# LiWentomng/OrientedRepPoints

Hardware: NVIDIA H100
Metric: 1024x1024 tiles/sec (higher is better)
Workload: dtype f16x3

## Files before the change

orientedreppoints_b200/_lib.py:

```python
import ctypes
import os

_HERE = os.path.dirname(os.path.abspath(__file__))
LIB_PATH = os.path.join(_HERE, "lib", "liborp_b200.so")

ORP_NMS_EXACT64, ORP_NMS_COMPAT32 = 0, 1
ORP_UNION_NAN_KEEPS, ORP_UNION_GUARD, ORP_UNION_NAN_SUPPRESSES, ORP_UNION_NAN_SUPPRESSES_ALL = 0, 1, 2, 3
ORP_ORDER_INDEX_ASC, ORP_ORDER_SCORE_DESC = 0, 1
ORP_MERGE_BAD_COUNT, ORP_MERGE_BAD_TILE, ORP_MERGE_ROWS_OVERFLOW = 1, 2, 4

_vp = ctypes.c_void_p
_i = ctypes.c_int
_f = ctypes.c_float
_d = ctypes.c_double


class NmsStats(ctypes.Structure):
    _fields_ = [("pairs_total", ctypes.c_int64), ("pairs_aabb", ctypes.c_int64),
                ("pairs_clipped", ctypes.c_int64), ("pairs_fp64", ctypes.c_int64),
                ("edges", ctypes.c_int64), ("suppressing", ctypes.c_int64), ("overflow", ctypes.c_int32),
                ("rounds", ctypes.c_int32), ("n", ctypes.c_int32)]

    def as_dict(self):
        return {k: int(getattr(self, k)) for k, _ in self._fields_}
# ... 101 lines not shown
    "orp_stem_s2d_u8_padded_bf16": (_i, [_vp, _i, _i, _i, _vp, _vp, _i, _vp, _vp, _vp]),
    "orp_stem_s2d_u8_padded_f16x3": (_i, [_vp, _i, _i, _i, _vp, _vp, _i, _vp, _vp, _vp]),
    "orp_patch_embed_rows_u8_padded_bf16": (_i, [_vp, _i, _i, _i, _vp, _vp, _i, _vp, _vp, _vp]),
    "orp_patch_embed_rows_u8_padded_f16x3": (_i, [_vp, _i, _i, _i, _vp, _vp, _i, _vp, _vp, _vp]),
    "orp_stem_s2d_u8_bf16": (_i, [_vp, _i, _i, _i, _vp, _vp, _i, _vp, _vp]),
    "orp_stem_conv_s2d_bf16": (_i, [_vp, _i, _i, _i, _vp, _vp, _i, _vp, _vp]),
    "orp_maxpool3x3s2_bf16": (_i, [_vp, _i, _i, _i, _i, _vp, _vp]),
    "orp_gn_stats_bf16": (_i, [_vp, _i, _i, _i, _i, _vp, _vp]),
    "orp_gn_apply_bf16_multi": (_i, [_i, _vp, _i, _i, _vp, _vp, _f, _i, _vp]),
}

DCNV2_SIGNATURES = {
    "orp_dcnv2_offset_mask": (_i, [_vp, ctypes.c_longlong, _vp, _vp, _vp]),
}

_LIB = None


class OrpError(RuntimeError):
    pass


def lib():
    global _LIB
    if _LIB is None:
        if not os.path.exists(LIB_PATH):
            raise OrpError(
                "liborp_b200.so not found at %s - build it with `python -m orientedreppoints_b200.build` "
                "(there is no CPU or PyTorch fallback for this path)" % LIB_PATH)
        l = ctypes.CDLL(LIB_PATH)
        for name, (res, args) in list(SIGNATURES.items()) + list(DCNV2_SIGNATURES.items()):
            fn = getattr(l, name)
            fn.restype = res
            fn.argtypes = args
        _LIB = l
    return _LIB


def check(rc, what=""):
    if rc != 0:
        msg = lib().orp_last_error()
        raise OrpError("%s failed (%d): %s" % (what, rc, msg.decode() if msg else ""))


def launch_count():
    return int(lib().orp_launch_count())
# ... 23 lines not shown
    v = ctypes.c_float(0)
    check(lib().orp_rnms_last_sweep_ms(ctypes.byref(v)), "orp_rnms_last_sweep_ms")
    return float(v.value)


def tc_timing_collect():
    ms, n, fl = ctypes.c_float(0), ctypes.c_int(0), ctypes.c_double(0)
    check(lib().orp_tc_timing_collect(ctypes.byref(ms), ctypes.byref(n), ctypes.byref(fl)), "orp_tc_timing_collect")
    return float(ms.value), int(n.value), float(fl.value)


def tc_last_plan():
    p = TcPlan()
    check(lib().orp_tc_last_plan(ctypes.byref(p)), "orp_tc_last_plan")
    return p.as_dict()


def tc_plan_for(problems, cout, cout_p, kh, kw, cin, stride, pad, *, bias=False, relu=0, out_f32=False, deform=False,
                split=False, residual=0, gn=False, stem=0, ksplit=1, sms=132):
    ph = 256
    arr = (TcProblem * len(problems))()
    for q, (n, h, w) in zip(arr, problems):
        q.x, q.N, q.H, q.W, q.out = ph, n, h, w, ph
        q.residual_bf16 = ph if residual == 1 else None
        q.residual_f32 = ph if residual == 2 else None
        q.offset = ph if deform else None
        q.gn_stats = ph if gn else None
    p = TcPlan()
    check(lib().orp_tc_plan_conv(len(problems), arr, ph, cout, cout_p, kh, kw, cin, stride, pad, ph if bias else None, 0,
                                 int(relu), int(out_f32), int(deform), int(split), stem, ksplit, sms, ctypes.byref(p)),
# ... 12 lines not shown
```

orientedreppoints_b200/build.py:

```python
import os
import subprocess
import sys
from concurrent.futures import ThreadPoolExecutor

HERE = os.path.dirname(os.path.abspath(__file__))
CSRC = os.path.join(HERE, "csrc")
OUT = os.path.join(HERE, "lib")
LIB = os.path.join(OUT, "liborp_b200.so")
NVCC = os.environ.get("NVCC", "/usr/local/cuda/bin/nvcc")
ARCH = ["-gencode", "arch=compute_90a,code=sm_90a"]
FLAGS = ["-O3", "-std=c++17", "-lineinfo", "-Xcompiler", "-fPIC", "--expt-relaxed-constexpr",
         "-Xptxas", "-v", "--threads", "2"]


def _sources():
    return sorted(os.path.join(CSRC, f) for f in os.listdir(CSRC) if f.endswith(".cu"))


def _headers():
    hs = [os.path.join(CSRC, f) for f in os.listdir(CSRC) if f.endswith((".cuh", ".h"))]
    hs.append(os.path.join(HERE, "..", "include", "orp_b200.h"))
    hs.append(os.path.join(HERE, "..", "include", "orp_b200_dcnv2.h"))
    return hs


def build(force=False, verbose=False):
    os.makedirs(OUT, exist_ok=True)
    objdir = os.path.join(OUT, "obj")
    os.makedirs(objdir, exist_ok=True)
    hdr_m = max(os.path.getmtime(h) for h in _headers())
    jobs = []
    objs = []
    for src in _sources():
        obj = os.path.join(objdir, os.path.basename(src)[:-3] + ".o")
        objs.append(obj)
        if force or not os.path.exists(obj) or os.path.getmtime(obj) < max(os.path.getmtime(src), hdr_m):
            jobs.append((src, obj))
# ... 30 lines not shown
```

orientedreppoints_b200/csrc/dense_tc.cu:

```cuda
#include <cuda.h>
#include <cuda_bf16.h>
#include <cuda_fp16.h>

#include <cstdlib>
#include <mutex>
#include <type_traits>

#include "common.cuh"
#include "wgmma.cuh"

namespace orp {
namespace {

constexpr int kMaxProb = 5;
constexpr int kStagesMax = 6;
constexpr int kBM = 128;
constexpr int kBK = 64;
constexpr int kABytes = kBM * kBK * 2;

struct FastDiv {
    uint32_t mul, shr, d;
    __host__ void set(uint32_t div)
    {
        d = div;
// ... 12 lines not shown
    int BW, BH, BI;
    int lbw, lbh;
    int tiles_w, tiles_h, tiles_i, tile_start;
    void *out;
    const __nv_bfloat16 *res;
    const float *res32;
    const __nv_bfloat16 *x;
    const float *offset;
    const float *mask;
    double *gn_stats;
};

struct alignas(64) TcParams {
    CUtensorMap tmA[kMaxProb];
    CUtensorMap tmB;
    CUtensorMap tmOut[kMaxProb];
    CUtensorMap tmRes[kMaxProb];
    CUtensorMap tmI;
    Problem prob[kMaxProb];
    int tma_epi, epi_bufs;
    int epi_merge;
    int ncat;
    int ksplit;
    FastDiv fd_ks;
    long long ks_stride;
    int b_resident;
    int res_mma;
    int gn_fused;
    int dcat;
    int split;
    float oscale;
    unsigned int *ovf;
    int nprob, num_m_tiles, n_tiles_n, num_tiles;
    FastDiv fd_ntn;
    int KH, KW, Cin, cin_blocks, stride, pad, Cout, relu;
    int s2d_stem;
    const float *bias;
};

__device__ __forceinline__ uint32_t smem_u32(const void *p) { return (uint32_t)__cvta_generic_to_shared(p); }

__device__ __forceinline__ void mbar_init(uint64_t *bar, uint32_t count)
{
    asm volatile("mbarrier.init.shared::cta.b64 [%0], %1;" ::"r"(smem_u32(bar)), "r"(count));
}
__device__ __forceinline__ void mbar_expect_tx(uint64_t *bar, uint32_t bytes)
{
    asm volatile("mbarrier.arrive.expect_tx.shared::cta.b64 _, [%0], %1;" ::"r"(smem_u32(bar)), "r"(bytes) : "memory");
// ... 31 lines not shown
        "cp.async.bulk.tensor.4d.shared::cluster.global.mbarrier::complete_tx::bytes [%0], [%1, {%3, %4, %5, %6}], [%2];"
        ::"r"(smem_u32(smem)), "l"(tm), "r"(smem_u32(bar)), "r"(c0), "r"(c1), "r"(c2), "r"(c3) : "memory");
}
__device__ __forceinline__ void tma_load_5d(void *smem, const CUtensorMap *tm, uint64_t *bar, int c0, int c1, int c2, int c3, int c4)
{
    asm volatile(
        "cp.async.bulk.tensor.5d.shared::cluster.global.mbarrier::complete_tx::bytes [%0], [%1, {%3, %4, %5, %6, %7}], [%2];"
        ::"r"(smem_u32(smem)), "l"(tm), "r"(smem_u32(bar)), "r"(c0), "r"(c1), "r"(c2), "r"(c3), "r"(c4) : "memory");
}
__device__ __forceinline__ void tma_load_2d(void *smem, const CUtensorMap *tm, uint64_t *bar, int c0, int c1)
{
    asm volatile(
        "cp.async.bulk.tensor.2d.shared::cluster.global.mbarrier::complete_tx::bytes [%0], [%1, {%3, %4}], [%2];"
        ::"r"(smem_u32(smem)), "l"(tm), "r"(smem_u32(bar)), "r"(c0), "r"(c1) : "memory");
}
__device__ __forceinline__ uint64_t make_desc_sw128(uint32_t smem_addr)
{
    uint64_t d = 0;
    d |= (uint64_t)((smem_addr >> 4) & 0x3FFF);
    d |= (uint64_t)1 << 16;
    d |= (uint64_t)(1024 >> 4) << 32;
    d |= (uint64_t)1 << 62;
    return d;
}
__device__ __forceinline__ uint4 lds128(uint32_t addr)
{
    uint4 v;
    asm volatile("ld.shared.v4.b32 {%0, %1, %2, %3}, [%4];" : "=r"(v.x), "=r"(v.y), "=r"(v.z), "=r"(v.w) : "r"(addr) : "memory");
    return v;
}
// ... 89 lines not shown
    uint32_t mt_u, nt_u;
    if (P.ksplit > 1) tile = (int)P.fd_ks.div((uint32_t)tile);
    P.fd_ntn.divmod((uint32_t)tile, mt_u, nt_u);
    nt = (int)nt_u;
    const int mt = (int)mt_u;
    pi = 0;
#pragma unroll
    for (int k = 1; k < kMaxProb; ++k)
        if (k < P.nprob && mt >= P.prob[k].tile_start) pi = k;
    const Problem &pr = P.prob[pi];
    const int local = mt - pr.tile_start;
    uint32_t rest, wb_u, ib_u, hb_u;
    pr.fd_tw.divmod((uint32_t)local, rest, wb_u);
    pr.fd_th.divmod(rest, ib_u, hb_u);
    wb = (int)wb_u; hb = (int)hb_u; ib = (int)ib_u;
}

struct IdentBlock { unsigned short v[64 * 64]; };
constexpr IdentBlock make_ident()
{
    IdentBlock b{};
    for (int i = 0; i < 64; ++i) b.v[i * 64 + i] = 0x3F80;
    return b;
}
__device__ IdentBlock g_ident = make_ident();
struct IdentBlocks16 { unsigned short v[16][64 * 64]; };
constexpr IdentBlocks16 make_ident16()
{
    IdentBlocks16 b{};
    for (int s = 0; s < 16; ++s)
// ... 51 lines not shown
template <int NG, bool BF16, int R, int G = 0>
__device__ __forceinline__ void wgmma_cols64(float (&acc)[R], uint64_t da, uint64_t db, uint32_t accumulate)
{
    wgmma_n<64, BF16>(acc_view<32 * G, 32>(acc), da, db + (uint64_t)(G * 512), accumulate);
    if constexpr (G + 1 < NG) wgmma_cols64<NG, BF16, R, G + 1>(acc, da, db, accumulate);
}

template <int BN, bool BF16>
__device__ __forceinline__ void wgmma_dcat(float (&acc)[BN / 2], uint64_t da, uint64_t db, uint32_t accumulate)
{
    if constexpr (BN == 256) {
        wgmma_n<128, BF16>(acc_view<0, 64>(acc), da, db, accumulate);
        wgmma_n<128, BF16>(acc_view<64, 64>(acc), da, db + (uint64_t)1024, accumulate);
    } else {
        wgmma_n<BN, BF16>(acc, da, db, accumulate);
    }
}

constexpr int kProducerRegs = 40;
constexpr int kConsumerRegs = 232;
constexpr int kWideConsumerRegs = 160;
constexpr int kWideProducerRegs = 96;

template <int BN, bool OUT_F32, bool DEFORM, bool SPLIT, int WALK>
__global__ void __launch_bounds__(DEFORM ? kConsumers + kDP : kConsumers + 128, 1)
conv_tc_kernel(const __grid_constant__ TcParams P, int stages)
{
    static_assert(WALK != kWalkNcat || (SPLIT && !DEFORM && !OUT_F32 && BN >= 64 && BN <= 128), "ncat: f16x3 TMA-epilogue layers, BN 64..128");
    static_assert(!DEFORM || (WALK == kWalkDcat) == SPLIT, "deformable: dcat exactly in f16x3");
    static_assert(DEFORM || WALK != kWalkDcat, "dcat is the deformable walk");
// ... 19 lines not shown
    const int kblocks_all = P.KH * P.KW * P.cin_blocks * kWTerms;
    uint8_t *ident = smem;
    if (P.res_mma) smem += 8192;
    uint8_t *bres = smem;
    if (P.b_resident) smem += (size_t)kblocks_all * kBBytes;
    constexpr int HC = BN < 64 ? BN : 64;
    constexpr int kPitch = HC * 2 + 16;
    uint8_t *stage_out = smem + (size_t)stages * kStageBytes;
    __shared__ uint64_t bars[2 * kStagesMax];
    __shared__ __align__(16) float s_bias[256];
    __shared__ uint64_t bres_bar;
    uint64_t *full = bars;
    uint64_t *empty = bars + kStagesMax;

    const int warp = threadIdx.x >> 5, lane = threadIdx.x & 31;

    if (warp == kConsumers / 32 && elect_one()) {
        if (!DEFORM) {
#pragma unroll 1
            for (int p = 0; p < P.nprob; ++p)
                asm volatile("prefetch.tensormap [%0];" ::"l"(&P.tmA[p]) : "memory");
        }
        asm volatile("prefetch.tensormap [%0];" ::"l"(&P.tmB) : "memory");
    }
    if (warp == 0) {
        if (elect_one()) {
            for (int s = 0; s < stages; ++s) {
                mbar_init(&full[s], DEFORM ? 1 + kDP / 32 : 1);
                mbar_init(&empty[s], kConsumers / 128);
            }
            mbar_init(&bres_bar, 1);
            asm volatile("fence.mbarrier_init.release.cluster;" ::: "memory");
        }
        __syncwarp();
    }
    __syncthreads();
    const int taps_per = (P.KH * P.KW) / (P.ksplit > 1 ? P.ksplit : 1);
    const int kblocks = taps_per * P.cin_blocks * (kKMode ? 3 : 1);
    asm volatile("griddepcontrol.launch_dependents;" ::: "memory");
    asm volatile("griddepcontrol.wait;" ::: "memory");

    if (warp < kConsumers / 32) {
        if constexpr (!DEFORM) setmaxnreg_inc<kConsumerRegs>();
        if constexpr (kFragEpi) setmaxnreg_inc<kWideConsumerRegs>();
        const int cw = warp >> 2;
        const uint32_t a_off = (uint32_t)cw * 8192u;
        const bool leader = (threadIdx.x & 127) == 0;
        float acc[kAccN / 2];
        Ring r(stages);
        const int q = warp & 3, wg = warp >> 2;
        const int et = threadIdx.x, nthr = kEpiThreads;
        const int bar_a = 1, bar_b = 3;
        const int ch0 = wg, chs = kWG;
        const int frow = cw * 64 + (warp & 3) * 16 + (lane >> 2), fcol = 2 * (lane & 3);
        const uint32_t s_acc_u = smem_u32(s_acc);
        auto bar_sync = [](int id, int n) { asm volatile("bar.sync %0, %1;" ::"r"(id), "r"(n) : "memory"); };
        int ob = 0;
        int bias_nt = -1;
        if ((P.b_resident || P.res_mma) && (int)blockIdx.x < P.num_tiles) mbar_wait(&bres_bar, 0);
        for (int tile = blockIdx.x; tile < P.num_tiles; tile += gridDim.x) {
            int res_groups = 0;
            if constexpr (WALK == kWalkKRes) {
                const int nt = tile - (int)P.fd_ntn.div((uint32_t)tile) * P.n_tiles_n;
                for (int g = 0; g < BN / 64 && nt * BN + g * 64 < P.Cout; ++g) ++res_groups;
            }
            const int tap_lo = ksplit_of(P, tile) * taps_per;
            KIter it(tap_lo + taps_per, P.cin_blocks, kKMode, tap_lo);
            int held = -1;
            auto release = [&](int next) {
                if (held >= 0 && leader) mbar_arrive(&empty[held]);
                held = next;
            };
            for (int kb = 0; kb < kblocks; ++kb, it.next()) {
                if constexpr (kFragEpi) {
                    wgmma_wait<0>();
                    release(-1);
                }
                mbar_wait(&full[r.stage], r.phase);
                const uint32_t sa = smem_u32(smem + (size_t)r.stage * kStageBytes);
                const uint64_t da = make_desc_sw128(sa + a_off);
                const int slab = (it.tap * P.cin_blocks + it.cb) * kWTerms + (it.term == 2 ? 1 : 0);
                wgmma_fence();
                if constexpr (WALK == kWalkNcat) {
                    const uint32_t sb = P.b_resident ? smem_u32(bres + (size_t)slab * kBBytes) : sa + 2 * kABytes;
                    const uint64_t dl = make_desc_sw128(sa + kABytes + a_off);
// ... 106 lines not shown
                            if (P.relu) { f0 = fmaxf(f0, 0.f); f1 = fmaxf(f1, 0.f); }
                            if (oterm == 0) amax[hr][i >> 2] = fmaxf(fmaxf(amax[hr][i >> 2], fabsf(f0)), fabsf(f1));
                            const __half2 h2 = __floats2half2_rn(f0, f1);
                            uint32_t v = *reinterpret_cast<const uint32_t *>(&h2);
                            if (oterm) {
                                const float2 hf = __half22float2(h2);
                                const __half2 l2 = __floats2half2_rn(f0 - hf.x, f1 - hf.y);
                                v = *reinterpret_cast<const uint32_t *>(&l2);
                            }
                            const uint32_t at = obase + (uint32_t)row * 128u + ((uint32_t)(i ^ (row & 7)) << 4) + (uint32_t)fcol * 2u;
                            asm volatile("st.shared.b32 [%0], %1;" ::"r"(at), "r"(v) : "memory");
                        }
                    }
                    asm volatile("fence.proxy.async.shared::cta;" ::: "memory");
                    bar_sync(bar_b, nthr);
                    if (io) {
                        asm volatile(
                            "cp.async.bulk.tensor.5d.global.shared::cta.bulk_group [%0, {%2, %3, %4, %5, %6}], [%1];"
                            ::"l"(&P.tmOut[pi]), "r"(obase), "r"(nt * BN + half * 64), "r"(oterm),
                              "r"(wb * pr.BW), "r"(hb * pr.BH), "r"(ib * pr.BI) : "memory");
                        asm volatile("cp.async.bulk.commit_group;" ::: "memory");
                    }
                    if (++ob == P.epi_bufs) ob = 0;
                }
#pragma unroll
                for (int hr = 0; hr < 2; ++hr)
#pragma unroll
                    for (int hc = 0; hc < 2; ++hc) {
                        float m = amax[hr][hc];
                        m = fmaxf(m, __shfl_xor_sync(0xffffffffu, m, 1));
                        m = fmaxf(m, __shfl_xor_sync(0xffffffffu, m, 2));
// ... 128 lines not shown
                                }
                                if (lane == c16) { gn_s = gs; gn_q = gq; }
                            }
                        }
                    }
                    if (P.gn_fused && oterm == 0 && lane < 8 && (chs == 1 || (lane >> 2) == wg)) {
                        const int n_img = ib * pr.BI + ((q * 32) >> (pr.lbw + pr.lbh));
                        if (n_img < pr.N) {
                            double *st = pr.gn_stats + ((size_t)n_img * 32 + (size_t)(nt * BN + half * 64) / 8 + lane) * 2;
                            atomicAdd(st, (double)gn_s);
                            atomicAdd(st + 1, (double)gn_q);
                        }
                    }
                    asm volatile("fence.proxy.async.shared::cta;" ::: "memory");
                    bar_sync(bar_b, nthr);
                    if (io) {
                        asm volatile(
                            "cp.async.bulk.tensor.5d.global.shared::cta.bulk_group [%0, {%2, %3, %4, %5, %6}], [%1];"
                            ::"l"(&P.tmOut[pi]), "r"(obuf_u + (uint32_t)ob * slot), "r"(nt * BN + half * 64), "r"(oterm),
                              "r"(wb * pr.BW), "r"(hb * pr.BH), "r"(ib * pr.BI) : "memory");
                        if (P.epi_merge)
                            asm volatile(
                                "cp.async.bulk.tensor.5d.global.shared::cta.bulk_group [%0, {%2, %3, %4, %5, %6}], [%1];"
                                ::"l"(&P.tmOut[pi]), "r"(obuf_u + (uint32_t)ob * slot + 16384u), "r"(nt * BN + half * 64), "r"(1),
                                  "r"(wb * pr.BW), "r"(hb * pr.BH), "r"(ib * pr.BI) : "memory");
                        asm volatile("cp.async.bulk.commit_group;" ::: "memory");
                    }
                    if (++ob == P.epi_bufs) ob = 0;
                }
                if (P.split && valid && amax > 65504.f) atomicAdd(P.ovf, 1u);
            } else {
// ... 77 lines not shown
                            } else {
                                const __nv_bfloat16 *e8 = reinterpret_cast<const __nv_bfloat16 *>(&u);
                                for (int j = 0; j < 8; ++j) if (cbase + k16 * 8 + j < P.Cout) op[j] = e8[j];
                            }
                        }
                    }
                    named_bar<1, kEpiThreads>();
                }
            }
        }
        if (P.tma_epi && et == 0) asm volatile("cp.async.bulk.wait_group 0;" ::: "memory");
    } else if (!DEFORM) {
        setmaxnreg_dec<kProducerRegs>();
        if (warp == kConsumers / 32 && elect_one()) {
            Ring r(stages);
            if ((P.b_resident || P.res_mma) && (int)blockIdx.x < P.num_tiles) {
                const int nt0 = blockIdx.x % P.n_tiles_n;
                mbar_expect_tx(&bres_bar, (uint32_t)((P.b_resident ? kblocks_all * kBBytes : 0) + (P.res_mma ? 8192 : 0)));
                if (P.res_mma) tma_load_2d(ident, &P.tmI, &bres_bar, 0, 0);
                if (P.b_resident)
                    for (int kb = 0; kb < kblocks_all; ++kb)
                        tma_load_2d(bres + (size_t)kb * kBBytes, &P.tmB, &bres_bar, kb * kBK, nt0 * BN);
            }
            for (int tile = blockIdx.x; tile < P.num_tiles; tile += gridDim.x) {
                int pi, wb, hb, ib, nt;
                decode_tile(P, tile, pi, wb, hb, ib, nt);
                const Problem &pr = P.prob[pi];
                const int w0 = wb * pr.BW * P.stride - P.pad, h0 = hb * pr.BH * P.stride - P.pad, i0 = ib * pr.BI;
                const int tap_lo = ksplit_of(P, tile) * taps_per;
                KIter it(tap_lo + taps_per, P.cin_blocks, kKMode, tap_lo);
                for (int j = 0; j < kblocks; ++j, it.next()) {
                    const int kh = it.tap / P.KW, kw = it.tap - kh * P.KW;
                    mbar_wait(&empty[r.stage], r.phase ^ 1);
                    uint8_t *sa = smem + (size_t)r.stage * kStageBytes;
                    const int wblk = ((it.tap * P.cin_blocks + it.cb) * kWTerms) * kBK;
                    if constexpr (WALK == kWalkNcat) {
                        mbar_expect_tx(&full[r.stage], 2 * kABytes + (P.b_resident ? 0 : 2 * kBBytes));
                        tma_load_5d(sa, &P.tmA[pi], &full[r.stage], it.cb * kBK, 0, w0 + kw, h0 + kh, i0);
                        tma_load_5d(sa + kABytes, &P.tmA[pi], &full[r.stage], it.cb * kBK, 1, w0 + kw, h0 + kh, i0);
// ... 19 lines not shown
                            r.next();
                        }
                }
            }
        }
    } else if (DEFORM) {
        __shared__ float4 s_w[2][128];
        __shared__ uint2 s_wh[2][128];
        __shared__ int4 s_o[2][128];
        if constexpr (kFragEpi) setmaxnreg_dec<kWideProducerRegs>();
        const int pt = threadIdx.x - kConsumers;
        auto load_b = [&](int stage, int tap, int cb, int nt) {
            uint8_t *sb = smem + (size_t)stage * kStageBytes + (P.dcat ? 2 * kABytes : kABytes);
            const int wblk = (tap * P.cin_blocks + cb) * (P.split ? 2 : 1) * kBK;
            mbar_expect_tx(&full[stage], P.dcat ? 2 * kBBytes : kBBytes);
            tma_load_2d(sb, &P.tmB, &full[stage], wblk, nt * BN);
            if (P.dcat) tma_load_2d(sb + kBBytes, &P.tmB, &full[stage], wblk + kBK, nt * BN);
        };
        Ring r(stages);
        int tb = 0;
        for (int tile = blockIdx.x; tile < P.num_tiles; tile += gridDim.x) {
            int pi, wb, hb, ib, nt;
            decode_tile(P, tile, pi, wb, hb, ib, nt);
            const Problem &pr = P.prob[pi];
            const int taps = P.KH * P.KW;
            for (int tap = 0; tap < taps; ++tap) {
                if (pt < 128) {
                    const int iw = pt & (pr.BW - 1), ih = (pt >> pr.lbw) & (pr.BH - 1), ii = pt >> (pr.lbw + pr.lbh);
                    const int w = wb * pr.BW + iw, h = hb * pr.BH + ih, n = ib * pr.BI + ii;
                    const bool valid = (w < pr.Wo) && (h < pr.Ho) && (n < pr.N);
                    const size_t opix = ((size_t)(valid ? n : 0) * pr.Ho + (valid ? h : 0)) * pr.Wo + (valid ? w : 0);
                    const float *offp = pr.offset + opix * (2 * taps);
                    const float *mskp = pr.mask ? pr.mask + opix * taps : nullptr;
                    const int cpp = P.Cin * (SPLIT ? 2 : 1);
                    const int img0 = (valid ? n : 0) * pr.H * pr.W * cpp;
                    const int kh = tap / P.KW, kw = tap - kh * P.KW;
// ... 125 lines not shown
                                    sts128(at, make_uint4(hi[0], hi[1], hi[2], hi[3]));
                                    sts128(at + kABytes, make_uint4(lo[0], lo[1], lo[2], lo[3]));
                                }
                            }
                        }
                        asm volatile("fence.proxy.async.shared::cta;" ::: "memory");
                        __syncwarp();
                        if ((pt & 31) == 0) mbar_arrive(&full[r.stage]);
                        r.next();
                    }
                }
                tb ^= 1;
            }
        }
    }
}

typedef CUresult (*EncodeTiledFn)(CUtensorMap *, CUtensorMapDataType, cuuint32_t, void *, const cuuint64_t *, const cuuint64_t *,
                                  const cuuint32_t *, const cuuint32_t *, CUtensorMapInterleave, CUtensorMapSwizzle,
                                  CUtensorMapL2promotion, CUtensorMapFloatOOBfill);

EncodeTiledFn encode_fn()
{
    static EncodeTiledFn fn = nullptr;
    static std::once_flag once;
    std::call_once(once, [] {
        void *p = nullptr;
        cudaDriverEntryPointQueryResult st;
        if (cudaGetDriverEntryPoint("cuTensorMapEncodeTiled", &p, cudaEnableDefault, &st) == cudaSuccess && st == cudaDriverEntryPointSuccess)
            fn = reinterpret_cast<EncodeTiledFn>(p);
    });
    return fn;
}

int pow2_floor(int v) { int p = 1; while (p * 2 <= v) p *= 2; return p; }

constexpr int kEvPool = 1024;
thread_local cudaEvent_t g_tc_ev[kEvPool][2];
thread_local int g_tc_ev_created = 0, g_tc_ev_used = 0;
thread_local double g_tc_flops = 0.0;
struct TcTrace { int nprob, N, H, W, Cin, Cout, K, stride, deform, BN, tiles, grid; double flops; };
thread_local TcTrace g_tc_trace[kEvPool];
thread_local orp_tc_plan g_tc_plan;
thread_local bool g_tc_plan_set = false;

constexpr int kSmemPerBlock = 227 * 1024;
constexpr int kStaticSmemPlain = 4096;
constexpr int kStaticSmemDeform = 14336;

struct ConvDesc {
    int nprob;
    const orp_tc_problem *probs;
    const void *w;
    int Cout, Cout_padded, KH, KW, Cin, stride, pad;
    const float *bias;
    int relu, out_f32, deform;
    int split;
    int wscale_log2;
    int stem;
// ... 122 lines not shown
    orp_tc_plan &r = pl.rep;
    r.BN = BN; r.stages = stages; r.grid = grid; r.num_tiles = num_tiles; r.n_tiles_n = n_tiles_n;
    r.ksplit = ksplit; r.nprob = nprob; r.Cout = d.Cout; r.Cout_padded = d.Cout_padded;
    r.split = d.split ? 1 : 0; r.deform = d.deform ? 1 : 0; r.out_f32 = d.out_f32 ? 1 : 0; r.stem = d.stem; r.relu = d.relu;
    r.bias = d.bias ? 1 : 0;
    for (int i = 0; i < nprob; ++i) {
        if (probs[i].residual_bf16) r.residual = 1;
        else if (probs[i].residual_f32) r.residual = 2;
        r.BW[i] = pl.prob[i].BW; r.BH[i] = pl.prob[i].BH; r.BI[i] = pl.prob[i].BI;
    }
    r.tma_epi = tma_epi; r.ncat = ncat; r.dcat = dcat; r.res_mma = res_mma; r.b_resident = b_resident;
    r.epi_merge = epi_merge; r.epi_bufs = epi_bufs; r.gn_fused = gn_fused; r.n_pair = n_pair;
    return ORP_OK;
}

int make_params(const ConvDesc &d, const ConvPlan &pl, TcParams &P)
{
    memset(&P, 0, sizeof(P));
    P.nprob = d.nprob; P.KH = d.KH; P.KW = d.KW; P.Cin = d.Cin; P.cin_blocks = (d.Cin + kBK - 1) / kBK;
    P.stride = d.stride; P.pad = d.pad;
    P.Cout = d.Cout; P.relu = d.relu; P.bias = d.bias; P.s2d_stem = (d.stem == 2) ? 1 : 0;
    P.split = d.split ? 1 : 0;
    P.oscale = d.split ? ldexpf(1.f, -d.wscale_log2) : 1.f;
    {
        void *ovf = nullptr;
        ORP_CUDA(cudaGetSymbolAddress(&ovf, g_f16_overflow));
        P.ovf = static_cast<unsigned int *>(ovf);
    }
    P.n_tiles_n = pl.rep.n_tiles_n / pl.rep.n_pair;
    P.fd_ntn.set((uint32_t)P.n_tiles_n);
    for (int i = 0; i < d.nprob; ++i) {
        const orp_tc_problem &q = d.probs[i];
        Problem &pr = P.prob[i];
        pr = pl.prob[i];
        pr.out = q.out; pr.res = static_cast<const __nv_bfloat16 *>(q.residual_bf16); pr.res32 = q.residual_f32;
        pr.x = static_cast<const __nv_bfloat16 *>(q.x); pr.offset = q.offset; pr.gn_stats = q.gn_stats; pr.mask = q.mask;
    }
    P.num_m_tiles = pl.num_m_tiles;
    P.num_tiles = pl.rep.num_tiles / pl.rep.n_pair;
    P.ksplit = d.ksplit;
    P.fd_ks.set((uint32_t)d.ksplit);
    P.ks_stride = (long long)P.prob[0].N * P.prob[0].Ho * P.prob[0].Wo * d.Cout;
    P.tma_epi = pl.rep.tma_epi; P.epi_bufs = pl.rep.epi_bufs; P.epi_merge = pl.rep.epi_merge; P.ncat = pl.rep.ncat;
    P.b_resident = pl.rep.b_resident; P.res_mma = pl.rep.res_mma; P.gn_fused = pl.rep.gn_fused; P.dcat = pl.rep.dcat;
    return ORP_OK;
}

int encode_maps(const ConvDesc &d, const ConvPlan &pl, TcParams &P)
{
    EncodeTiledFn enc = encode_fn();
    if (!enc) return fail(ORP_ECUDA, "conv2d_tc: cuTensorMapEncodeTiled unavailable");
    const CUtensorMapDataType dt16 = d.split ? CU_TENSOR_MAP_DATA_TYPE_FLOAT16 : CU_TENSOR_MAP_DATA_TYPE_BFLOAT16;
    const int T = d.split ? 2 : 1, Cin = d.Cin, Cout = d.Cout, stride = d.stride;
    if (!d.deform) {
        for (int i = 0; i < d.nprob; ++i) {
            const orp_tc_problem &q = d.probs[i];
            const Problem &pr = P.prob[i];
            cuuint64_t gdim[5] = {(cuuint64_t)Cin, (cuuint64_t)T, (cuuint64_t)q.W, (cuuint64_t)q.H, (cuuint64_t)q.N};
            cuuint64_t gstr[4] = {(cuuint64_t)Cin * 2, (cuuint64_t)Cin * 2 * T, (cuuint64_t)q.W * Cin * 2 * T,
// ... 10 lines not shown
                             CU_TENSOR_MAP_INTERLEAVE_NONE, CU_TENSOR_MAP_SWIZZLE_128B, CU_TENSOR_MAP_L2_PROMOTION_L2_128B,
                             CU_TENSOR_MAP_FLOAT_OOB_FILL_NONE);
            if (r != CUDA_SUCCESS) return fail(ORP_ECUDA, "conv2d_tc: cuTensorMapEncodeTiled(A) failed");
        }
    }
    {
        const cuuint64_t K = (cuuint64_t)d.KH * d.KW * T * P.cin_blocks * kBK;
        cuuint64_t gdim[2] = {K, (cuuint64_t)d.Cout_padded};
        cuuint64_t gstr[1] = {K * 2};
        cuuint32_t box[2] = {(cuuint32_t)kBK, (cuuint32_t)pl.kbn};
        cuuint32_t estr[2] = {1, 1};
        CUresult r = enc(&P.tmB, dt16, 2, const_cast<void *>(d.w), gdim, gstr, box, estr,
                         CU_TENSOR_MAP_INTERLEAVE_NONE, CU_TENSOR_MAP_SWIZZLE_128B, CU_TENSOR_MAP_L2_PROMOTION_L2_256B,
                         CU_TENSOR_MAP_FLOAT_OOB_FILL_NONE);
        if (r != CUDA_SUCCESS) return fail(ORP_ECUDA, "conv2d_tc: cuTensorMapEncodeTiled(B) failed");
    }
    if (P.res_mma) {
        void *ident_ptr = nullptr;
        if (d.split) {
            ORP_CUDA(cudaGetSymbolAddress(&ident_ptr, g_ident16));
            ident_ptr = static_cast<char *>(ident_ptr) + (size_t)d.wscale_log2 * 8192;
        } else {
            ORP_CUDA(cudaGetSymbolAddress(&ident_ptr, g_ident));
        }
        cuuint64_t gdim[2] = {64, 64};
        cuuint64_t gstr[1] = {128};
        cuuint32_t box[2] = {64, 64};
        cuuint32_t estr[2] = {1, 1};
        CUresult r = enc(&P.tmI, dt16, 2, ident_ptr, gdim, gstr, box, estr, CU_TENSOR_MAP_INTERLEAVE_NONE,
                         CU_TENSOR_MAP_SWIZZLE_128B, CU_TENSOR_MAP_L2_PROMOTION_NONE, CU_TENSOR_MAP_FLOAT_OOB_FILL_NONE);
// ... 11 lines not shown
                             CU_TENSOR_MAP_INTERLEAVE_NONE, CU_TENSOR_MAP_SWIZZLE_128B, CU_TENSOR_MAP_L2_PROMOTION_NONE,
                             CU_TENSOR_MAP_FLOAT_OOB_FILL_NONE);
            if (r != CUDA_SUCCESS) return fail(ORP_ECUDA, "conv2d_tc: cuTensorMapEncodeTiled(out) failed");
            if (pr.res) {
                r = enc(&P.tmRes[i], dt16, 5, const_cast<__nv_bfloat16 *>(pr.res), gdim, gstr, box, estr,
                        CU_TENSOR_MAP_INTERLEAVE_NONE, CU_TENSOR_MAP_SWIZZLE_128B, CU_TENSOR_MAP_L2_PROMOTION_L2_128B,
                        CU_TENSOR_MAP_FLOAT_OOB_FILL_NONE);
                if (r != CUDA_SUCCESS) return fail(ORP_ECUDA, "conv2d_tc: cuTensorMapEncodeTiled(residual) failed");
            }
        }
    }
    return ORP_OK;
}

template <int BN, bool OUT_F32, bool DEFORM, bool SPLIT, int WALK>
int launch_tc(const TcParams &P, int stages, int grid, cudaStream_t st, int extra_bytes)
{
    constexpr bool kCat = WALK == kWalkNcat || WALK == kWalkDcat;
    const int smem = dyn_smem_bytes(stage_bytes(BN, kCat, P.b_resident), stages, extra_bytes, frag_epilogue(BN, DEFORM));
    auto kern = conv_tc_kernel<BN, OUT_F32, DEFORM, SPLIT, WALK>;
    static int smem_max = -1;
    if (smem_max < 0) {
        cudaFuncAttributes fa;
        ORP_CUDA(cudaFuncGetAttributes(&fa, kern));
        ORP_CUDA(cudaFuncSetAttribute(kern, cudaFuncAttributeMaxDynamicSharedMemorySize, kSmemPerBlock - (int)fa.sharedSizeBytes));
        smem_max = kSmemPerBlock - (int)fa.sharedSizeBytes;
    }
    if (smem > smem_max) {
        char need[32];
        snprintf(need, sizeof(need), "%d", smem);
        return fail(ORP_EINVAL, "conv2d_tc: the plan's %s bytes of dynamic shared memory do not fit beside the static shared memory of %s",
                    need, __PRETTY_FUNCTION__);
    }
    int slot = -1;
    if (g_timing && g_tc_ev_used < kEvPool) {
        slot = g_tc_ev_used++;
        if (slot >= g_tc_ev_created) {
            ORP_CUDA(cudaEventCreate(&g_tc_ev[slot][0]));
            ORP_CUDA(cudaEventCreate(&g_tc_ev[slot][1]));
            g_tc_ev_created = slot + 1;
        }
        ORP_CUDA(cudaEventRecord(g_tc_ev[slot][0], st));
        double fl = 0;
        for (int i = 0; i < P.nprob; ++i)
            fl += 2.0 * P.prob[i].N * P.prob[i].Ho * P.prob[i].Wo * (double)P.Cout *
                  (P.s2d_stem ? 147.0 : (double)P.KH * P.KW * P.Cin);
        g_tc_flops += fl;
        g_tc_trace[slot] = TcTrace{P.nprob, P.prob[0].N, P.prob[0].H, P.prob[0].W, P.Cin, P.Cout, P.KH, P.stride, DEFORM ? 1 : 0,
                                   BN, P.num_tiles, grid, fl};
    }
    {
        cudaLaunchConfig_t cfg;
        memset(&cfg, 0, sizeof(cfg));
        cfg.gridDim = dim3((unsigned)grid);
        cfg.blockDim = dim3(DEFORM ? (unsigned)(kConsumers + kDP) : (unsigned)(kConsumers + 128));
        cfg.dynamicSmemBytes = smem;
        cfg.stream = st;
        cudaLaunchAttribute at[1];
        at[0].id = cudaLaunchAttributeProgrammaticStreamSerialization;
        at[0].val.programmaticStreamSerializationAllowed = 1;
        cfg.attrs = at;
        cfg.numAttrs = 1;
        ORP_CUDA(cudaLaunchKernelEx(&cfg, kern, P, stages));
    }
    ORP_LAUNCHED();
    if (slot >= 0) ORP_CUDA(cudaEventRecord(g_tc_ev[slot][1], st));
    return ORP_OK;
}

template <int BN, bool OUT_F32, bool DEFORM>
int launch_plan(const TcParams &P, int stages, int grid, cudaStream_t st, int extra_bytes)
{
    if constexpr (DEFORM) {
        if (P.dcat != P.split || P.ncat || P.res_mma) return fail(ORP_EINVAL, "conv2d_tc: deformable plan outside dcat == split");
        if constexpr (frag_epilogue(BN, true)) {
            if (!P.split || OUT_F32 || !P.tma_epi || P.epi_merge || P.gn_fused || P.relu == 2)
                return fail(ORP_EINVAL, "conv2d_tc: deformable N-tile pair outside f16x3 with an unmerged TMA epilogue and no GELU");
            return launch_tc<BN, false, true, true, kWalkDcat>(P, stages, grid, st, extra_bytes);
        } else {
// ... 149 lines not shown
}

using namespace orp;

extern "C" int orp_tc_timing_collect(float *total_ms, int *launches, double *flops)
{
    if (!total_ms || !launches || !flops) return fail(ORP_EINVAL, "orp_tc_timing_collect: null");
    float sum = 0.f;
    for (int i = 0; i < g_tc_ev_used; ++i) {
        float ms = 0.f;
        ORP_CUDA(cudaEventSynchronize(g_tc_ev[i][1]));
        ORP_CUDA(cudaEventElapsedTime(&ms, g_tc_ev[i][0], g_tc_ev[i][1]));
        sum += ms;
        if (getenv("ORP_TC_TRACE")) {
            const TcTrace &t = g_tc_trace[i];
            fprintf(stderr, "tc[%3d] np=%d N=%d %4dx%-4d Cin=%4d Cout=%4d k=%d s=%d dcn=%d BN=%3d tiles=%5d grid=%3d  %8.1f us  %7.1f TFLOP/s\n",
                    i, t.nprob, t.N, t.H, t.W, t.Cin, t.Cout, t.K, t.stride, t.deform, t.BN, t.tiles, t.grid, ms * 1e3,
                    t.flops / (ms * 1e-3) / 1e12);
        }
    }
    *total_ms = sum; *launches = g_tc_ev_used; *flops = g_tc_flops;
    g_tc_ev_used = 0; g_tc_flops = 0.0;
    return ORP_OK;
}

extern "C" int orp_tc_last_plan(orp_tc_plan *out)
{
    if (!out) return fail(ORP_EINVAL, "orp_tc_last_plan: null");
    if (!g_tc_plan_set) return fail(ORP_EINVAL, "orp_tc_last_plan: no tensor-core convolution launched on this thread");
    *out = g_tc_plan;
    return ORP_OK;
}

extern "C" int orp_tc_plan_conv(int nprob, const orp_tc_problem *probs, const void *w, int Cout, int Cout_padded, int KH, int KW,
                                int Cin, int stride, int pad, const float *bias, int wscale_log2, int relu, int out_f32, int deform,
                                int split, int stem, int ksplit, int sms, orp_tc_plan *out)
{
    if (!out || sms < 1 || (stem != 0 && stem != 2)) return fail(ORP_EINVAL, "orp_tc_plan_conv: bad arguments");
    split = split ? 1 : 0;
    orp_tc_problem q;
    ConvDesc d;
    int rc = ORP_OK;
    if (stem == 2 || ksplit > 1) {
        if (nprob != 1 || !probs || deform || out_f32 || (stem == 2 && ksplit > 1))
            return fail(ORP_EINVAL, "orp_tc_plan_conv: the stem and split-K plan one problem with a 16-bit output");
        int Ho, Wo;
        rc = stem == 2 ? stem_desc(probs->x, probs->N, probs->H, probs->W, w, bias, relu, probs->out, split, wscale_log2, q, d)
// ... 96 lines not shown
```

Before: 323.2.

## Pair CTAs into 2-clusters and multicast weight tiles for deformable convs

For deformable tensor-core convolutions, CTAs are launched as clusters of two that take adjacent M tiles sharing the same N tile. Each CTA TMA-loads half of the weight tile and multicasts it to both, and the empty barriers count arrivals from both CTAs so neither overwrites a stage its partner still reads. The goal is to halve weight (B) traffic per CTA and its L2 load. The cost is cross-CTA synchronisation coupling, padded tile counts that need out-of-range store guards, and an occupancy check that falls back to unpaired launches.

Measured after the change: 323.7 (median of 6 runs). Within noise of the previous version (+0.1%).

```diff
diff --git a/include/orp_b200_tc_pairs.h b/include/orp_b200_tc_pairs.h
--- /dev/null
+++ b/include/orp_b200_tc_pairs.h
@@ -0,0 +1,15 @@
+#ifndef ORP_B200_TC_PAIRS_H_
+#define ORP_B200_TC_PAIRS_H_
+
+#ifdef __cplusplus
+extern "C" {
+#endif
+
+int orp_tc_last_cluster(int *size);
+void orp_tc_pair_ctas(int on);
+
+#ifdef __cplusplus
+}
+#endif
+
+#endif
diff --git a/orientedreppoints_b200/_lib.py b/orientedreppoints_b200/_lib.py
--- a/orientedreppoints_b200/_lib.py
+++ b/orientedreppoints_b200/_lib.py
@@ -139,6 +139,11 @@
     "orp_dcnv2_offset_mask": (_i, [_vp, ctypes.c_longlong, _vp, _vp, _vp]),
 }
 
+TC_PAIR_SIGNATURES = {
+    "orp_tc_last_cluster": (_i, [ctypes.POINTER(_i)]),
+    "orp_tc_pair_ctas": (None, [_i]),
+}
+
 _LIB = None
 
 
@@ -154,7 +159,7 @@
                 "liborp_b200.so not found at %s - build it with `python -m orientedreppoints_b200.build` "
                 "(there is no CPU or PyTorch fallback for this path)" % LIB_PATH)
         l = ctypes.CDLL(LIB_PATH)
-        for name, (res, args) in list(SIGNATURES.items()) + list(DCNV2_SIGNATURES.items()):
+        for name, (res, args) in list(SIGNATURES.items()) + list(DCNV2_SIGNATURES.items()) + list(TC_PAIR_SIGNATURES.items()):
             fn = getattr(l, name)
             fn.restype = res
             fn.argtypes = args
@@ -208,6 +213,16 @@
     p = TcPlan()
     check(lib().orp_tc_last_plan(ctypes.byref(p)), "orp_tc_last_plan")
     return p.as_dict()
+
+
+def tc_last_cluster():
+    v = ctypes.c_int(0)
+    check(lib().orp_tc_last_cluster(ctypes.byref(v)), "orp_tc_last_cluster")
+    return int(v.value)
+
+
+def tc_pair_ctas(on):
+    lib().orp_tc_pair_ctas(1 if on else 0)
 
 
 def tc_plan_for(problems, cout, cout_p, kh, kw, cin, stride, pad, *, bias=False, relu=0, out_f32=False, deform=False,
diff --git a/orientedreppoints_b200/build.py b/orientedreppoints_b200/build.py
--- a/orientedreppoints_b200/build.py
+++ b/orientedreppoints_b200/build.py
@@ -21,6 +21,7 @@
     hs = [os.path.join(CSRC, f) for f in os.listdir(CSRC) if f.endswith((".cuh", ".h"))]
     hs.append(os.path.join(HERE, "..", "include", "orp_b200.h"))
     hs.append(os.path.join(HERE, "..", "include", "orp_b200_dcnv2.h"))
+    hs.append(os.path.join(HERE, "..", "include", "orp_b200_tc_pairs.h"))
     return hs
 
 
diff --git a/orientedreppoints_b200/csrc/dense_tc.cu b/orientedreppoints_b200/csrc/dense_tc.cu
--- a/orientedreppoints_b200/csrc/dense_tc.cu
+++ b/orientedreppoints_b200/csrc/dense_tc.cu
@@ -7,6 +7,7 @@
 #include <type_traits>
 
 #include "common.cuh"
+#include "../../include/orp_b200_tc_pairs.h"
 #include "wgmma.cuh"
 
 namespace orp {
@@ -50,6 +51,7 @@
 struct alignas(64) TcParams {
     CUtensorMap tmA[kMaxProb];
     CUtensorMap tmB;
+    CUtensorMap tmBh;
     CUtensorMap tmOut[kMaxProb];
     CUtensorMap tmRes[kMaxProb];
     CUtensorMap tmI;
@@ -68,6 +70,8 @@
     float oscale;
     unsigned int *ovf;
     int nprob, num_m_tiles, n_tiles_n, num_tiles;
+    int pair;
+    int tile_end;
     FastDiv fd_ntn;
     int KH, KW, Cin, cin_blocks, stride, pad, Cout, relu;
     int s2d_stem;
@@ -129,6 +133,25 @@
         "cp.async.bulk.tensor.2d.shared::cluster.global.mbarrier::complete_tx::bytes [%0], [%1, {%3, %4}], [%2];"
         ::"r"(smem_u32(smem)), "l"(tm), "r"(smem_u32(bar)), "r"(c0), "r"(c1) : "memory");
 }
+__device__ __forceinline__ void tma_load_2d_mc(void *smem, const CUtensorMap *tm, uint64_t *bar, int c0, int c1, uint16_t mask)
+{
+    asm volatile(
+        "cp.async.bulk.tensor.2d.shared::cluster.global.mbarrier::complete_tx::bytes.multicast::cluster [%0], [%1, {%3, %4}], [%2], %5;"
+        ::"r"(smem_u32(smem)), "l"(tm), "r"(smem_u32(bar)), "r"(c0), "r"(c1), "h"(mask) : "memory");
+}
+__device__ __forceinline__ void mbar_arrive_cluster(uint64_t *bar, uint32_t rank)
+{
+    asm volatile(
+        "{\n\t"
+        ".reg .b32 ra;\n\t"
+        "mapa.shared::cluster.u32 ra, %0, %1;\n\t"
+        "mbarrier.arrive.shared::cluster.b64 _, [ra];\n\t"
+        "}" ::"r"(smem_u32(bar)), "r"(rank) : "memory");
+}
+__device__ __forceinline__ void cluster_sync()
+{
+    asm volatile("barrier.cluster.arrive.release;\n\tbarrier.cluster.wait.acquire;" ::: "memory");
+}
 __device__ __forceinline__ uint64_t make_desc_sw128(uint32_t smem_addr)
 {
     uint64_t d = 0;
@@ -248,6 +271,21 @@
     pr.fd_tw.divmod((uint32_t)local, rest, wb_u);
     pr.fd_th.divmod(rest, ib_u, hb_u);
     wb = (int)wb_u; hb = (int)hb_u; ib = (int)ib_u;
+}
+
+__device__ __forceinline__ int pair_tile(const TcParams &P, uint32_t slot)
+{
+    uint32_t mp, nt;
+    P.fd_ntn.divmod(slot, mp, nt);
+    return (int)((2 * mp + (blockIdx.x & 1)) * (uint32_t)P.n_tiles_n + nt);
+}
+__device__ __forceinline__ int first_tile(const TcParams &P, bool pair) { return pair ? pair_tile(P, blockIdx.x >> 1) : (int)blockIdx.x; }
+__device__ __forceinline__ int next_tile(const TcParams &P, int tile, bool pair)
+{
+    if (!pair) return tile + (int)gridDim.x;
+    uint32_t mt, nt;
+    P.fd_ntn.divmod((uint32_t)tile, mt, nt);
+    return pair_tile(P, (mt >> 1) * (uint32_t)P.n_tiles_n + nt + (gridDim.x >> 1));
 }
 
 struct IdentBlock { unsigned short v[64 * 64]; };
@@ -329,6 +367,17 @@
         wgmma_n<128, BF16>(acc_view<64, 64>(acc), da, db + (uint64_t)1024, accumulate);
     } else {
         wgmma_n<BN, BF16>(acc, da, db, accumulate);
+    }
+}
+
+template <int BN>
+__device__ __forceinline__ void load_w(const TcParams &P, bool pair, uint8_t *dst, uint64_t *bar, int k, int row0)
+{
+    if (pair) {
+        const int h = (int)(blockIdx.x & 1) * (BN / 2);
+        tma_load_2d_mc(dst + h * kBK * 2, &P.tmBh, bar, k, row0 + h, 0x3);
+    } else {
+        tma_load_2d(dst, &P.tmB, bar, k, row0);
     }
 }
 
@@ -378,6 +427,7 @@
     uint64_t *empty = bars + kStagesMax;
 
     const int warp = threadIdx.x >> 5, lane = threadIdx.x & 31;
+    const bool pair = DEFORM && P.pair;
 
     if (warp == kConsumers / 32 && elect_one()) {
         if (!DEFORM) {
@@ -391,7 +441,7 @@
         if (elect_one()) {
             for (int s = 0; s < stages; ++s) {
                 mbar_init(&full[s], DEFORM ? 1 + kDP / 32 : 1);
-                mbar_init(&empty[s], kConsumers / 128);
+                mbar_init(&empty[s], (kConsumers / 128) * (pair ? 2 : 1));
             }
             mbar_init(&bres_bar, 1);
             asm volatile("fence.mbarrier_init.release.cluster;" ::: "memory");
@@ -399,6 +449,7 @@
         __syncwarp();
     }
     __syncthreads();
+    if (pair) cluster_sync();
     const int taps_per = (P.KH * P.KW) / (P.ksplit > 1 ? P.ksplit : 1);
     const int kblocks = taps_per * P.cin_blocks * (kKMode ? 3 : 1);
     asm volatile("griddepcontrol.launch_dependents;" ::: "memory");
@@ -421,8 +472,8 @@
         auto bar_sync = [](int id, int n) { asm volatile("bar.sync %0, %1;" ::"r"(id), "r"(n) : "memory"); };
         int ob = 0;
         int bias_nt = -1;
-        if ((P.b_resident || P.res_mma) && (int)blockIdx.x < P.num_tiles) mbar_wait(&bres_bar, 0);
-        for (int tile = blockIdx.x; tile < P.num_tiles; tile += gridDim.x) {
+        if ((P.b_resident || P.res_mma) && first_tile(P, pair) < P.tile_end) mbar_wait(&bres_bar, 0);
+        for (int tile = first_tile(P, pair); tile < P.tile_end; tile = next_tile(P, tile, pair)) {
             int res_groups = 0;
             if constexpr (WALK == kWalkKRes) {
                 const int nt = tile - (int)P.fd_ntn.div((uint32_t)tile) * P.n_tiles_n;
@@ -432,7 +483,10 @@
             KIter it(tap_lo + taps_per, P.cin_blocks, kKMode, tap_lo);
             int held = -1;
             auto release = [&](int next) {
-                if (held >= 0 && leader) mbar_arrive(&empty[held]);
+                if (held >= 0 && leader) {
+                    mbar_arrive(&empty[held]);
+                    if (pair) mbar_arrive_cluster(&empty[held], (blockIdx.x & 1) ^ 1);
+                }
                 held = next;
             };
             for (int kb = 0; kb < kblocks; ++kb, it.next()) {
@@ -569,7 +623,7 @@
                     }
                     asm volatile("fence.proxy.async.shared::cta;" ::: "memory");
                     bar_sync(bar_b, nthr);
-                    if (io) {
+                    if (io && tile < P.num_tiles) {
                         asm volatile(
                             "cp.async.bulk.tensor.5d.global.shared::cta.bulk_group [%0, {%2, %3, %4, %5, %6}], [%1];"
                             ::"l"(&P.tmOut[pi]), "r"(obase), "r"(nt * BN + half * 64), "r"(oterm),
@@ -728,7 +782,7 @@
                     }
                     asm volatile("fence.proxy.async.shared::cta;" ::: "memory");
                     bar_sync(bar_b, nthr);
-                    if (io) {
+                    if (io && tile < P.num_tiles) {
                         asm volatile(
                             "cp.async.bulk.tensor.5d.global.shared::cta.bulk_group [%0, {%2, %3, %4, %5, %6}], [%1];"
                             ::"l"(&P.tmOut[pi]), "r"(obuf_u + (uint32_t)ob * slot), "r"(nt * BN + half * 64), "r"(oterm),
@@ -836,7 +890,7 @@
         setmaxnreg_dec<kProducerRegs>();
         if (warp == kConsumers / 32 && elect_one()) {
             Ring r(stages);
-            if ((P.b_resident || P.res_mma) && (int)blockIdx.x < P.num_tiles) {
+            if ((P.b_resident || P.res_mma) && first_tile(P, pair) < P.tile_end) {
                 const int nt0 = blockIdx.x % P.n_tiles_n;
                 mbar_expect_tx(&bres_bar, (uint32_t)((P.b_resident ? kblocks_all * kBBytes : 0) + (P.res_mma ? 8192 : 0)));
                 if (P.res_mma) tma_load_2d(ident, &P.tmI, &bres_bar, 0, 0);
@@ -844,7 +898,7 @@
                     for (int kb = 0; kb < kblocks_all; ++kb)
                         tma_load_2d(bres + (size_t)kb * kBBytes, &P.tmB, &bres_bar, kb * kBK, nt0 * BN);
             }
-            for (int tile = blockIdx.x; tile < P.num_tiles; tile += gridDim.x) {
+            for (int tile = first_tile(P, pair); tile < P.tile_end; tile = next_tile(P, tile, pair)) {
                 int pi, wb, hb, ib, nt;
                 decode_tile(P, tile, pi, wb, hb, ib, nt);
                 const Problem &pr = P.prob[pi];
@@ -894,12 +948,12 @@
             uint8_t *sb = smem + (size_t)stage * kStageBytes + (P.dcat ? 2 * kABytes : kABytes);
             const int wblk = (tap * P.cin_blocks + cb) * (P.split ? 2 : 1) * kBK;
             mbar_expect_tx(&full[stage], P.dcat ? 2 * kBBytes : kBBytes);
-            tma_load_2d(sb, &P.tmB, &full[stage], wblk, nt * BN);
-            if (P.dcat) tma_load_2d(sb + kBBytes, &P.tmB, &full[stage], wblk + kBK, nt * BN);
+            load_w<BN>(P, pair, sb, &full[stage], wblk, nt * BN);
+            if (P.dcat) load_w<BN>(P, pair, sb + kBBytes, &full[stage], wblk + kBK, nt * BN);
         };
         Ring r(stages);
         int tb = 0;
-        for (int tile = blockIdx.x; tile < P.num_tiles; tile += gridDim.x) {
+        for (int tile = first_tile(P, pair); tile < P.tile_end; tile = next_tile(P, tile, pair)) {
             int pi, wb, hb, ib, nt;
             decode_tile(P, tile, pi, wb, hb, ib, nt);
             const Problem &pr = P.prob[pi];
@@ -1055,6 +1109,7 @@
             }
         }
     }
+    if (pair) cluster_sync();
 }
 
 typedef CUresult (*EncodeTiledFn)(CUtensorMap *, CUtensorMapDataType, cuuint32_t, void *, const cuuint64_t *, const cuuint64_t *,
@@ -1080,10 +1135,12 @@
 thread_local cudaEvent_t g_tc_ev[kEvPool][2];
 thread_local int g_tc_ev_created = 0, g_tc_ev_used = 0;
 thread_local double g_tc_flops = 0.0;
-struct TcTrace { int nprob, N, H, W, Cin, Cout, K, stride, deform, BN, tiles, grid; double flops; };
+struct TcTrace { int nprob, N, H, W, Cin, Cout, K, stride, deform, BN, tiles, grid, pair; double flops; };
 thread_local TcTrace g_tc_trace[kEvPool];
 thread_local orp_tc_plan g_tc_plan;
 thread_local bool g_tc_plan_set = false;
+thread_local bool g_tc_pairing = true;
+thread_local int g_tc_last_cluster = 0;
 
 constexpr int kSmemPerBlock = 227 * 1024;
 constexpr int kStaticSmemPlain = 4096;
@@ -1236,6 +1293,19 @@
     return ORP_OK;
 }
 
+bool pairable(const orp_tc_plan &r)
+{
+    if (!r.deform || r.ksplit != 1 || r.grid % 2) return false;
+    const int tiles = r.num_tiles / r.n_pair, ntn = r.n_tiles_n / r.n_pair, m = tiles / ntn;
+    return ceil_div(2 * ceil_div(m, 2) * ntn, r.grid) == ceil_div(tiles, r.grid);
+}
+
+void set_pairing(TcParams &P, bool pair)
+{
+    P.pair = pair ? 1 : 0;
+    P.tile_end = pair ? 2 * ceil_div(P.num_m_tiles, 2) * P.n_tiles_n : P.num_tiles;
+}
+
 int make_params(const ConvDesc &d, const ConvPlan &pl, TcParams &P)
 {
     memset(&P, 0, sizeof(P));
@@ -1265,6 +1335,7 @@
     P.ks_stride = (long long)P.prob[0].N * P.prob[0].Ho * P.prob[0].Wo * d.Cout;
     P.tma_epi = pl.rep.tma_epi; P.epi_bufs = pl.rep.epi_bufs; P.epi_merge = pl.rep.epi_merge; P.ncat = pl.rep.ncat;
     P.b_resident = pl.rep.b_resident; P.res_mma = pl.rep.res_mma; P.gn_fused = pl.rep.gn_fused; P.dcat = pl.rep.dcat;
+    set_pairing(P, pairable(pl.rep));
     return ORP_OK;
 }
 
@@ -1305,6 +1376,12 @@
                          CU_TENSOR_MAP_INTERLEAVE_NONE, CU_TENSOR_MAP_SWIZZLE_128B, CU_TENSOR_MAP_L2_PROMOTION_L2_256B,
                          CU_TENSOR_MAP_FLOAT_OOB_FILL_NONE);
         if (r != CUDA_SUCCESS) return fail(ORP_ECUDA, "conv2d_tc: cuTensorMapEncodeTiled(B) failed");
+        if (P.pair) {
+            box[1] = (cuuint32_t)(pl.kbn / 2);
+            r = enc(&P.tmBh, dt16, 2, const_cast<void *>(d.w), gdim, gstr, box, estr, CU_TENSOR_MAP_INTERLEAVE_NONE,
+                    CU_TENSOR_MAP_SWIZZLE_128B, CU_TENSOR_MAP_L2_PROMOTION_L2_256B, CU_TENSOR_MAP_FLOAT_OOB_FILL_NONE);
+            if (r != CUDA_SUCCESS) return fail(ORP_ECUDA, "conv2d_tc: cuTensorMapEncodeTiled(B half) failed");
+        }
     }
     if (P.res_mma) {
         void *ident_ptr = nullptr;
@@ -1346,7 +1423,7 @@
 }
 
 template <int BN, bool OUT_F32, bool DEFORM, bool SPLIT, int WALK>
-int launch_tc(const TcParams &P, int stages, int grid, cudaStream_t st, int extra_bytes)
+int launch_tc(TcParams P, int stages, int grid, cudaStream_t st, int extra_bytes)
 {
     constexpr bool kCat = WALK == kWalkNcat || WALK == kWalkDcat;
     const int smem = dyn_smem_bytes(stage_bytes(BN, kCat, P.b_resident), stages, extra_bytes, frag_epilogue(BN, DEFORM));
@@ -1364,6 +1441,33 @@
         return fail(ORP_EINVAL, "conv2d_tc: the plan's %s bytes of dynamic shared memory do not fit beside the static shared memory of %s",
                     need, __PRETTY_FUNCTION__);
     }
+    cudaLaunchConfig_t cfg;
+    memset(&cfg, 0, sizeof(cfg));
+    cfg.gridDim = dim3((unsigned)grid);
+    cfg.blockDim = dim3(DEFORM ? (unsigned)(kConsumers + kDP) : (unsigned)(kConsumers + 128));
+    cfg.dynamicSmemBytes = smem;
+    cfg.stream = st;
+    cudaLaunchAttribute at[2];
+    at[0].id = cudaLaunchAttributeClusterDimension;
+    at[0].val.clusterDim.x = 2; at[0].val.clusterDim.y = 1; at[0].val.clusterDim.z = 1;
+    if (P.pair && g_tc_pairing) {
+        static std::mutex mu;
+        static int known = 0, known_smem[16], known_pairs[16];
+        std::lock_guard<std::mutex> lock(mu);
+        int pairs = -1;
+        for (int i = 0; i < known; ++i)
+            if (known_smem[i] == smem) pairs = known_pairs[i];
+        if (pairs < 0) {
+            cfg.attrs = at;
+            cfg.numAttrs = 1;
+            ORP_CUDA(cudaOccupancyMaxActiveClusters(&pairs, kern, &cfg));
+            if (known < 16) { known_smem[known] = smem; known_pairs[known] = pairs; ++known; }
+        }
+        if (pairs < grid / 2) set_pairing(P, false);
+    } else {
+        set_pairing(P, false);
+    }
+    g_tc_last_cluster = P.pair ? 2 : 1;
     int slot = -1;
     if (g_timing && g_tc_ev_used < kEvPool) {
         slot = g_tc_ev_used++;
@@ -1379,22 +1483,13 @@
                   (P.s2d_stem ? 147.0 : (double)P.KH * P.KW * P.Cin);
         g_tc_flops += fl;
         g_tc_trace[slot] = TcTrace{P.nprob, P.prob[0].N, P.prob[0].H, P.prob[0].W, P.Cin, P.Cout, P.KH, P.stride, DEFORM ? 1 : 0,
-                                   BN, P.num_tiles, grid, fl};
-    }
-    {
-        cudaLaunchConfig_t cfg;
-        memset(&cfg, 0, sizeof(cfg));
-        cfg.gridDim = dim3((unsigned)grid);
-        cfg.blockDim = dim3(DEFORM ? (unsigned)(kConsumers + kDP) : (unsigned)(kConsumers + 128));
-        cfg.dynamicSmemBytes = smem;
-        cfg.stream = st;
-        cudaLaunchAttribute at[1];
-        at[0].id = cudaLaunchAttributeProgrammaticStreamSerialization;
-        at[0].val.programmaticStreamSerializationAllowed = 1;
-        cfg.attrs = at;
-        cfg.numAttrs = 1;
-        ORP_CUDA(cudaLaunchKernelEx(&cfg, kern, P, stages));
-    }
+                                   BN, P.num_tiles, grid, P.pair, fl};
+    }
+    at[1].id = cudaLaunchAttributeProgrammaticStreamSerialization;
+    at[1].val.programmaticStreamSerializationAllowed = 1;
+    cfg.attrs = P.pair ? at : at + 1;
+    cfg.numAttrs = P.pair ? 2 : 1;
+    ORP_CUDA(cudaLaunchKernelEx(&cfg, kern, P, stages));
     ORP_LAUNCHED();
     if (slot >= 0) ORP_CUDA(cudaEventRecord(g_tc_ev[slot][1], st));
     return ORP_OK;
@@ -1574,8 +1669,9 @@
         sum += ms;
         if (getenv("ORP_TC_TRACE")) {
             const TcTrace &t = g_tc_trace[i];
-            fprintf(stderr, "tc[%3d] np=%d N=%d %4dx%-4d Cin=%4d Cout=%4d k=%d s=%d dcn=%d BN=%3d tiles=%5d grid=%3d  %8.1f us  %7.1f TFLOP/s\n",
-                    i, t.nprob, t.N, t.H, t.W, t.Cin, t.Cout, t.K, t.stride, t.deform, t.BN, t.tiles, t.grid, ms * 1e3,
+            fprintf(stderr, "tc[%3d] np=%d N=%d %4dx%-4d Cin=%4d Cout=%4d k=%d s=%d dcn=%d BN=%3d tiles=%5d grid=%3d%s  %8.1f us  %7.1f TFLOP/s\n",
+                    i, t.nprob, t.N, t.H, t.W, t.Cin, t.Cout, t.K, t.stride, t.deform, t.BN, t.tiles, t.grid, t.pair ? " pairs" : "      ",
+                    ms * 1e3,
                     t.flops / (ms * 1e-3) / 1e12);
         }
     }
@@ -1591,6 +1687,16 @@
     *out = g_tc_plan;
     return ORP_OK;
 }
+
+extern "C" int orp_tc_last_cluster(int *size)
+{
+    if (!size) return fail(ORP_EINVAL, "orp_tc_last_cluster: null");
+    if (!g_tc_plan_set) return fail(ORP_EINVAL, "orp_tc_last_cluster: no tensor-core convolution launched on this thread");
+    *size = g_tc_last_cluster;
+    return ORP_OK;
+}
+
+extern "C" void orp_tc_pair_ctas(int on) { g_tc_pairing = on != 0; }
 
 extern "C" int orp_tc_plan_conv(int nprob, const orp_tc_problem *probs, const void *w, int Cout, int Cout_padded, int KH, int KW,
                                 int Cin, int stride, int pad, const float *bias, int wscale_log2, int relu, int out_f32, int deform,
```
